# ViliamVadocz/takzero

Measured on AMD Instinct MI355X. Metric: mcts_simulations_per_s, higher is better.
Workload: dtype f16

## Files before the change

takzero_amd/csrc/tz_capi.hip:

```cpp
#include <algorithm>
#include <array>
#include <cmath>
#include <cstdlib>
#include <cstring>
#include <vector>

#include "tz_math.h"
#include "tz_nn.h"

struct tz_search {
    SearchDev d;
    tz_net* net = nullptr;
    int device = 0;
    hipStream_t stream = nullptr;
    bool own_stream = false;
    float* noise_dev = nullptr;
    int noise_cap = 0;
    uint16_t* act_dev = nullptr;
    int32_t* i32_dev = nullptr;
    int8_t* i8_dev = nullptr;
    tz_root_info* info_dev = nullptr;
    void* child_dev = nullptr;
    size_t child_cap = 0;
    hipGraphExec_t graph[2] = {nullptr, nullptr};
    int warm[2] = {0, 0};
    uint64_t graph_gen[2] = {0, 0};
    bool use_graph = true;
    uint64_t sim_index = 0;
    LeafBatchDev lb = {};
    size_t lb_slots = 0;
    std::vector<std::array<hipEvent_t, 4>> batch_events;
    double batch_ms[3] = {0.0, 0.0, 0.0};
    uint64_t batch_rounds = 0;
    bool profile = false;
    double tree_ms = 0.0;
    uint64_t steps = 0;
    std::vector<std::pair<hipEvent_t, hipEvent_t>> tree_events;
};

namespace {

int default_capacity(int n) { return n <= 3 ? 16384 : n == 4 ? 65536 : n == 5 ? 262144 : 524288; }
// ... 31 lines not shown
        (void)hipEventDestroy(ev.second);
    }
    s->tree_events.clear();
    if (s->net) {
        for (auto& ev : s->net->conv_events) {
            float ms = 0.f;
            if (hipEventElapsedTime(&ms, ev.first, ev.second) == hipSuccess) s->net->conv_ms += ms;
            (void)hipEventDestroy(ev.first);
            (void)hipEventDestroy(ev.second);
        }
        s->net->conv_events.clear();
    }
    return TZ_OK;
}

int one_simulation_eager(tz_search* s, bool from_start, bool profile);

int one_simulation(tz_search* s, bool from_start) {
    const int gi = from_start ? 1 : 0;
    s->sim_index++;
    const bool sample = s->profile && (s->sim_index % 8 == 0);
    if (!s->use_graph || sample || s->warm[gi] < 2) {
        s->warm[gi]++;
        return one_simulation_eager(s, from_start, sample);
    }
    if (s->graph[gi] && s->net && s->graph_gen[gi] != s->net->weights_gen) {
        (void)hipGraphExecDestroy(s->graph[gi]);
        s->graph[gi] = nullptr;
    }
    if (!s->graph[gi]) {
        hipGraph_t g = nullptr;
        TZ_HIP(hipStreamBeginCapture(s->stream, hipStreamCaptureModeThreadLocal));
        const int rc = one_simulation_eager(s, from_start, false);
        const hipError_t e = hipStreamEndCapture(s->stream, &g);
        if (rc) {
            if (g) (void)hipGraphDestroy(g);
            return rc;
        }
        if (e != hipSuccess) return tz_fail(TZ_EDEVICE, std::string("hipStreamEndCapture: ") + hipGetErrorString(e));
        const hipError_t ei = hipGraphInstantiate(&s->graph[gi], g, nullptr, nullptr, 0);
        (void)hipGraphDestroy(g);
        if (ei != hipSuccess) return tz_fail(TZ_EDEVICE, std::string("hipGraphInstantiate: ") + hipGetErrorString(ei));
        s->graph_gen[gi] = s->net ? s->net->weights_gen : 0;
    }
    TZ_HIP(hipGraphLaunch(s->graph[gi], s->stream));
    return TZ_OK;
}

int one_simulation_eager(tz_search* s, bool from_start, bool profile) {
    int rc;
    hipEvent_t e0 = nullptr, e1 = nullptr, e2 = nullptr, e3 = nullptr;
    const bool saved_net_profile = s->net ? s->net->profile : false;
    if (s->net) s->net->profile = profile;
    struct Restore {
        tz_search* s;
        bool v;
        ~Restore() {
            if (s->net) s->net->profile = v;
        }
    } restore{s, saved_net_profile};
    if (profile) {
        TZ_HIP(hipEventCreate(&e0));
        TZ_HIP(hipEventCreate(&e1));
        TZ_HIP(hipEventCreate(&e2));
        TZ_HIP(hipEventCreate(&e3));
        TZ_HIP(hipEventRecord(e0, s->stream));
    }
    if ((rc = tz_tree_descend(s->d, from_start, s->stream))) return rc;
    if ((rc = tz_tree_compact_leaves(s->d, s->stream))) return rc;
    if (profile) TZ_HIP(hipEventRecord(e1, s->stream));
    NetOut out{nullptr, 0, nullptr, nullptr};
    if (s->d.agent_kind == TZ_AGENT_NET) {
        if ((rc = tz_net_forward_device(s->net, s->d.leaf_env, s->d.nn_game, s->d.nn_count, 0, s->d.batch, s->stream, &out)))
            return rc;
    }
    if (profile) TZ_HIP(hipEventRecord(e2, s->stream));
    if ((rc = tz_tree_expand(s->d, out, s->stream))) return rc;
    if (profile) {
        TZ_HIP(hipEventRecord(e3, s->stream));
        s->tree_events.push_back({e0, e1});
        s->tree_events.push_back({e2, e3});
        s->steps++;
    }
    return TZ_OK;
}

int ensure_noise(tz_search* s, int amax) {
    if ((size_t)amax * s->d.batch <= (size_t)s->noise_cap) return TZ_OK;
    if (s->noise_dev) (void)hipFree(s->noise_dev);
    s->noise_dev = nullptr;
    TZ_HIP(hipMalloc(&s->noise_dev, (size_t)amax * s->d.batch * sizeof(float)));
    s->noise_cap = amax * s->d.batch;
    return TZ_OK;
}

// ... 56 lines not shown
    s->batch_events.clear();
    return TZ_OK;
}

int one_batch_round(tz_search* s) {
    int rc;
    std::array<hipEvent_t, 4> ev = {nullptr, nullptr, nullptr, nullptr};
    if (s->profile) {
        for (hipEvent_t& e : ev) TZ_HIP(hipEventCreate(&e));
        s->batch_events.push_back(ev);
        TZ_HIP(hipEventRecord(ev[0], s->stream));
    }
    if ((rc = tz_tree_descend_batch(s->d, s->lb, s->stream))) return rc;
    if ((rc = tz_tree_compact_batch(s->d, s->lb, s->stream))) return rc;
    if (s->profile) TZ_HIP(hipEventRecord(ev[1], s->stream));
    NetOut out{nullptr, 0, nullptr, nullptr};
    if (s->d.agent_kind == TZ_AGENT_NET) {
        if ((rc = tz_net_forward_device(s->net, s->lb.env, s->lb.index, s->d.nn_count, 0, s->d.batch * s->lb.leaves, s->stream, &out)))
            return rc;
    }
    if (s->profile) TZ_HIP(hipEventRecord(ev[2], s->stream));
    if ((rc = tz_tree_expand_batch(s->d, s->lb, out, s->stream))) return rc;
    if (s->profile) TZ_HIP(hipEventRecord(ev[3], s->stream));
    return TZ_OK;
}

int ensure_child(tz_search* s, size_t bytes) {
    if (bytes <= s->child_cap) return TZ_OK;
    if (s->child_dev) (void)hipFree(s->child_dev);
    s->child_dev = nullptr;
    TZ_HIP(hipMalloc(&s->child_dev, bytes));
// ... 5 lines not shown

extern "C" {

int tz_search_create(tz_net* net, int agent_kind, int batch, int board_n, int half_komi, int node_capacity,
                     tz_search** out) {
    if (!out || batch <= 0 || board_n < 3 || board_n > 6) return tz_fail(TZ_EINVAL, "tz_search_create: bad argument");
    if (agent_kind != TZ_AGENT_NET && agent_kind != TZ_AGENT_DUMMY && agent_kind != TZ_AGENT_SIMPLE)
        return tz_fail(TZ_EINVAL, "tz_search_create: unknown agent kind");
    if (agent_kind == TZ_AGENT_NET && (!net || net->n != board_n))
        return tz_fail(TZ_EINVAL, "tz_search_create: TZ_AGENT_NET needs a network of the same board size");
    int ndev = 0;
    if (hipGetDeviceCount(&ndev) != hipSuccess || ndev == 0)
        return tz_fail(TZ_EDEVICE, "tz_search_create: no HIP device available (the HIP path has no CPU fallback)");
    tz_search* s = new tz_search();
    s->use_graph = getenv("TZ_NO_GRAPH") == nullptr;
    s->net = agent_kind == TZ_AGENT_NET ? net : nullptr;
    s->device = s->net ? s->net->device : 0;
    TZ_HIP(hipSetDevice(s->device));
    if (s->net) {
        s->stream = s->net->stream;
    } else {
        TZ_HIP(hipStreamCreate(&s->stream));
        s->own_stream = true;
    }
    SearchDev& d = s->d;
    memset(&d, 0, sizeof d);
    d.batch = batch;
    d.n = board_n;
    d.half_komi = half_komi;
    d.cap = node_capacity > 0 ? node_capacity : default_capacity(board_n);
// ... 12 lines not shown
    rc |= dev_alloc(&d.t.child0, nodes);
    rc |= dev_alloc(&d.t.nchild, nodes);
    rc |= dev_alloc(&d.t.action, nodes);
    rc |= dev_alloc(&d.bank, batch);
    rc |= dev_alloc(&d.alloc, batch);
    rc |= dev_alloc(&d.env, batch);
    rc |= dev_alloc(&d.betas, batch);
    rc |= dev_alloc(&d.traj, (size_t)batch * TZ_MAX_DEPTH);
    rc |= dev_alloc(&d.traj_len, batch);
    rc |= dev_alloc(&d.start_node, batch);
    rc |= dev_alloc(&d.leaf_kind, batch);
    rc |= dev_alloc(&d.leaf_nact, batch);
    rc |= dev_alloc(&d.leaf_act, (size_t)batch * d.max_actions);
    rc |= dev_alloc(&d.leaf_env, batch);
    rc |= dev_alloc(&d.nn_game, batch);
    rc |= dev_alloc(&d.nn_count, 1);
    rc |= dev_alloc(&d.bfs_src, (size_t)batch * d.cap);
    rc |= dev_alloc(&d.counters, 3);
    rc |= dev_alloc(&d.error_flag, 1);
    rc |= dev_alloc(&d.term_reason, batch);
    rc |= dev_alloc(&d.term_winner, batch);
    rc |= dev_alloc(&s->act_dev, batch);
    rc |= dev_alloc(&s->i32_dev, batch);
    rc |= dev_alloc(&s->i8_dev, batch);
    rc |= dev_alloc(&s->info_dev, batch);
    if (rc) {
        tz_search_destroy(s);
        return tz_fail(TZ_ENOMEM, "tz_search_create: device allocation failed (lower node_capacity or batch)");
    }
    TZ_HIP(hipMemsetAsync(d.bank, 0, batch, s->stream));
    TZ_HIP(hipMemsetAsync(d.env, 0, (size_t)batch * sizeof(tz_state), s->stream));
    TZ_HIP(hipMemsetAsync(d.leaf_env, 0, (size_t)batch * sizeof(tz_state), s->stream));
    TZ_HIP(hipMemsetAsync(d.betas, 0, batch * sizeof(float), s->stream));
    TZ_HIP(hipMemsetAsync(d.start_node, 0, batch * sizeof(int32_t), s->stream));
    TZ_HIP(hipMemsetAsync(d.counters, 0, 3 * sizeof(unsigned long long), s->stream));
    TZ_HIP(hipMemsetAsync(d.error_flag, 0, 4, s->stream));
    TZ_HIP(hipMemsetAsync(d.nn_count, 0, 4, s->stream));
    if (s->net && (rc = tz_net_ensure_batch(s->net, batch))) {
        tz_search_destroy(s);
        return rc;
    }
    if ((rc = tz_tree_restart(d, nullptr, nullptr, true, false, s->stream))) {
        tz_search_destroy(s);
        return rc;
    }
    TZ_HIP(hipStreamSynchronize(s->stream));
    *out = s;
    return TZ_OK;
}

int tz_search_destroy(tz_search* s) {
    if (!s) return TZ_OK;
    (void)hipSetDevice(s->device);
    if (s->stream) (void)hipStreamSynchronize(s->stream);
    drain_profile(s);
    for (int i = 0; i < 2; i++)
        if (s->graph[i]) (void)hipGraphExecDestroy(s->graph[i]);
    SearchDev& d = s->d;
    void* ptrs[] = {d.t.eval_tag, d.t.eval_bits, d.t.visits, d.t.prob, d.t.logit, d.t.std_dev, d.t.child0, d.t.nchild,
                    d.t.action, d.bank, d.alloc, d.env, d.betas, d.traj, d.traj_len, d.start_node, d.leaf_kind,
                    d.leaf_nact, d.leaf_act, d.leaf_env, d.nn_game, d.nn_count, d.bfs_src, d.counters, d.error_flag,
                    d.term_reason, d.term_winner,
                    s->noise_dev, s->act_dev, s->i32_dev, s->i8_dev, s->info_dev, s->child_dev};
    for (void* p : ptrs)
        if (p) (void)hipFree(p);
    free_leaf_batch(s);
    drain_batch_profile(s);
    if (s->own_stream && s->stream) (void)hipStreamDestroy(s->stream);
    delete s;
    return TZ_OK;
}

int tz_search_set_positions(tz_search* s, int count, const int32_t* game_idx, const tz_state* states) {
    if (!s || count < 0 || (count && (!game_idx || !states))) return tz_fail(TZ_EINVAL, "tz_search_set_positions: bad argument");
    if (count == 0) return TZ_OK;
    TZ_HIP(hipSetDevice(s->device));
// ... 24 lines not shown
    if (!s || !opening_choice) return tz_fail(TZ_EINVAL, "tz_search_new_openings: null argument");
    TZ_HIP(hipSetDevice(s->device));
    for (int g = 0; g < s->d.batch; g++)
        if (opening_choice[g] < 0 || opening_choice[g] >= 16) return tz_fail(TZ_EINVAL, "opening choice must be in [0,16)");
    TZ_HIP(hipMemcpyAsync(s->i32_dev, opening_choice, s->d.batch * sizeof(int32_t), hipMemcpyHostToDevice, s->stream));
    int rc = tz_tree_restart(s->d, s->i32_dev, nullptr, true, true, s->stream);
    if (rc) return rc;
    TZ_HIP(hipStreamSynchronize(s->stream));
    return TZ_OK;
}

int tz_search_simulate(tz_search* s, const float* betas, int n_sims) {
    if (!s || !betas || n_sims < 0) return tz_fail(TZ_EINVAL, "tz_search_simulate: bad argument");
    TZ_HIP(hipSetDevice(s->device));
    TZ_HIP(hipMemcpyAsync(s->d.betas, betas, s->d.batch * sizeof(float), hipMemcpyHostToDevice, s->stream));
    for (int i = 0; i < n_sims; i++) {
        int rc = one_simulation(s, false);
        if (rc) return rc;
    }
    int rc = check_error_flag(s);
    drain_profile(s);
    return rc;
}

int tz_search_simulate_batch(tz_search* s, const float* betas, int leaves, int rounds) {
    if (!s || !betas || leaves < 1 || rounds < 0) return tz_fail(TZ_EINVAL, "tz_search_simulate_batch: bad argument");
    if ((long long)s->d.batch * leaves > TZ_SIMULATE_BATCH_MAX_SLOTS)
        return tz_fail(TZ_EINVAL, "tz_search_simulate_batch: batch * leaves exceeds TZ_SIMULATE_BATCH_MAX_SLOTS");
    TZ_HIP(hipSetDevice(s->device));
    int rc = ensure_leaf_batch(s, leaves);
    if (rc) return rc;
    TZ_HIP(hipMemcpyAsync(s->d.betas, betas, s->d.batch * sizeof(float), hipMemcpyHostToDevice, s->stream));
    for (int i = 0; i < rounds; i++)
        if ((rc = one_batch_round(s))) return rc;
    rc = check_error_flag(s);
    drain_batch_profile(s);
    return rc;
}

int tz_search_set_selection(tz_search* s, int rule) {
    if (!s) return tz_fail(TZ_EINVAL, "tz_search_set_selection: null argument");
    if (rule != TZ_SELECT_PUCT && rule != TZ_SELECT_UCT && rule != TZ_SELECT_IMPROVED)
        return tz_fail(TZ_EINVAL, "tz_search_set_selection: unknown selection rule");
    TZ_HIP(hipSetDevice(s->device));
    TZ_HIP(hipStreamSynchronize(s->stream));
    for (int i = 0; i < 2; i++) {
        if (s->graph[i]) (void)hipGraphExecDestroy(s->graph[i]);
        s->graph[i] = nullptr;
        s->warm[i] = 0;
    }
    s->d.select_rule = rule;
    return TZ_OK;
}

int tz_search_get_selection(tz_search* s, int* rule_out) {
    if (!s || !rule_out) return tz_fail(TZ_EINVAL, "tz_search_get_selection: null argument");
    *rule_out = s->d.select_rule;
    return TZ_OK;
}

int tz_search_batch_profile(tz_search* s, double* forward_ms, double* net_ms, double* backward_ms, uint64_t* rounds) {
// ... 444 lines not shown
```

takzero_amd/csrc/tz_engine.h:

```cpp
#pragma once
#include <hip/hip_runtime.h>
#include <stdint.h>

#include <string>
#include <vector>

#include "../../include/takzero_hip.h"

#define TZ_MAX_DEPTH 512

void tz_set_error(const std::string& msg);
int tz_fail(int code, const std::string& msg);
#define TZ_HIP(call)                                                                              \
    do {                                                                                          \
        hipError_t _e = (call);                                                                   \
        if (_e != hipSuccess)                                                                     \
            return tz_fail(TZ_EDEVICE, std::string(#call) + ": " + hipGetErrorString(_e));       \
    } while (0)

struct TreeArrays {
    uint8_t* eval_tag;
    uint32_t* eval_bits;
    uint32_t* visits;
    float* prob;
// ... 9 lines not shown
    int strict_capacity;
    int select_rule;
    TreeArrays t;
    uint8_t* bank;
    uint32_t* alloc;
    tz_state* env;
    float* betas;
    uint32_t* traj;
    uint32_t* traj_len;
    int32_t* start_node;
    uint8_t* leaf_kind;
    uint16_t* leaf_nact;
    uint16_t* leaf_act;
    tz_state* leaf_env;
    int32_t* nn_game;
    int32_t* nn_count;
    uint32_t* bfs_src;
    unsigned long long* counters;
    int32_t* error_flag;
    int8_t* term_reason;
    uint8_t* term_winner;
};

struct LeafBatchDev {
    int leaves;
    tz_state* env;
    uint16_t* act;
    uint16_t* nact;
    uint32_t* traj;
    uint32_t* traj_len;
// ... 1 lines not shown
    float* prob;
    float* value;
    float* variance;
    uint8_t* bad;
    int32_t* count;
    int32_t* forwards;
    int32_t* offset;
    int32_t* index;
};

struct NetOut {
    const float* policy;
    int policy_stride;
    const float* value;
    const float* variance;
};

int tz_tree_descend(const SearchDev& s, bool from_start_nodes, hipStream_t st);
int tz_tree_compact_leaves(const SearchDev& s, hipStream_t st);
int tz_tree_expand(const SearchDev& s, const NetOut& out, hipStream_t st);
int tz_tree_apply_noise(const SearchDev& s, const float* noise_dev, int amax, float ratio, hipStream_t st);
int tz_tree_root_info(const SearchDev& s, tz_root_info* out_dev, hipStream_t st);
int tz_tree_root_children(const SearchDev& s, int amax, uint16_t* move_idx, uint32_t* visits, uint8_t* eval_tag,
                          uint32_t* eval_bits, float* logit, float* prob, float* std_dev, hipStream_t st);
int tz_tree_node(const SearchDev& s, int game, const uint16_t* path_dev, int len, uint32_t* out_words, int* status, int amax,
                 uint16_t* move_idx, uint32_t* visits, uint8_t* eval_tag, uint32_t* eval_bits, float* logit, float* prob, float* std_dev,
                 hipStream_t st);
int tz_tree_select_best(const SearchDev& s, uint16_t* out_dev, hipStream_t st);
int tz_tree_step(const SearchDev& s, const uint16_t* actions_dev, hipStream_t st);
int tz_tree_restart(const SearchDev& s, const int32_t* choice_dev, int8_t* terminal_dev, bool force_all,
                    bool with_opening_moves, hipStream_t st);
int tz_tree_reset_games(const SearchDev& s, const int32_t* idx_dev, int count, hipStream_t st);
int tz_tree_set_start_children(const SearchDev& s, const int32_t* child_index_dev, hipStream_t st);
int tz_tree_gumbel_root_fixup(const SearchDev& s, hipStream_t st);
int tz_tree_principal_variation(const SearchDev& s, int game, uint16_t* moves_dev, int cap, int* len_dev, hipStream_t st);
// ... 5 lines not shown
```

takzero_amd/csrc/tz_nn.h:

```cpp
#pragma once
#include <string>
#include <vector>

#include "tz_engine.h"
#include "tz_ot.h"

struct ConvW {
    int taps = 0, cin = 0, cin_pad = 0, cout = 0, cout_pad = 0;
    uint16_t* w_mfma = nullptr;
    uint16_t* w_lo = nullptr;
    unsigned char* w8 = nullptr;
    float c8_scale = 0.0f;
    float* w_f32 = nullptr;
    float* bias = nullptr;
};

struct tz_net {
    int n = 0, nn = 0, arch = 0, device = 0, precision = 0, blocks = 0;
    int cin = 0, cin_pad = 0, pol_ch = 0, pol_stride = 0, ppt = 0;
    bool loaded = false, has_rnd = false, has_hash = false;
    TensorStore store;
    uint64_t weights_gen = 0;
    ConvW conv_in, policy;
    std::vector<ConvW> res;
// ... 25 lines not shown
    hipStream_t stream = nullptr;
    void* dbg_buf = nullptr;
    int dbg_groups = 0;
    void* eval_host = nullptr;
    void* eval_dev = nullptr;
    size_t eval_bytes = 0;
    hipEvent_t ev0 = nullptr, ev1 = nullptr;
    std::vector<std::pair<hipEvent_t, hipEvent_t>> conv_events;
    bool profile = false;
    double conv_ms = 0.0;
    uint64_t conv_launches = 0;
};

int tz_net_ensure_batch(tz_net* net, int batch);
int tz_net_forward_device(tz_net* net, const tz_state* states_dev, const int32_t* game_index_dev,
                          const int32_t* count_dev, int count_host, int max_positions, hipStream_t st, NetOut* out);
int tz_nn_encode_planes(int n, int cin, const tz_state* states_dev, int count, float* planes_dev, hipStream_t st);
```

takzero_amd/csrc/tz_nn.hip:

```cpp
#include "tz_nn.h"
#include "tz_fp8.h"
#include "tz_fp6.h"
#include <type_traits>
#include "tz_ot.h"

#include <algorithm>
#include <cmath>
#include <cstdio>
#include <cstdlib>
#include <cstring>
#include <atomic>
#include <map>
#include <memory>
#include <mutex>
#include <thread>

int tz_nn_launch_split(int sp, int n, const void* net_args, int max_positions, hipStream_t st);
int tz_nn_launch_c6(int n, const void* net_args, int max_positions, hipStream_t st);
size_t tz_nn_c6_seed_bytes(int n, int max_positions);

namespace {

typedef float f32x4 __attribute__((ext_vector_type(4)));
typedef unsigned int u32x4 __attribute__((ext_vector_type(4)));
// ... 2346 lines not shown
    float ss = 0.f;
    for (int sq = 0; sq < NN; sq++) ss += part[sq];
#pragma unroll
    for (int k = 0; k < PER; k++) {
        const int i = l + k * 64;
        if (i < out_stride) out[(size_t)pos * out_stride + i] = (ET)(i < in_size ? x[k] / ss : 0.f);
    }
}

__global__ __launch_bounds__(64) void rnd_finish_kernel(const float* learn, const float* target, const float* ube,
                                                        const int32_t* count_dev, int count_host, int dim, int stride,
                                                        float rmin, float rmax, float* variance) {
    const int count = count_dev ? *count_dev : count_host;
    const int pos = blockIdx.x, l = threadIdx.x;
    if (pos >= count) return;
    float s = 0.f;
    for (int i = l; i < dim; i += 64) {
        const float d = learn[(size_t)pos * stride + i] - target[(size_t)pos * stride + i];
        s += d * d;
    }
    for (int d = 32; d >= 1; d >>= 1) s += __shfl_xor(s, d);
    if (l == 0) {
        float norm = (s - rmin) / (rmax - rmin);
        norm = fminf(fmaxf(norm, 0.f), 1.f) * 4.0f;
        variance[pos] = fminf(fmaxf(fmaxf(expf(ube[pos]), norm), 0.f), 4.f);
    }
}

__global__ void plain_variance_kernel(const float* ube, const float* local, const int32_t* count_dev, int count_host,
                                      float* variance) {
    const int count = count_dev ? *count_dev : count_host;
    const int pos = blockIdx.x * blockDim.x + threadIdx.x;
    if (pos >= count) return;
    const float loc = local ? local[pos] : 0.f;
    variance[pos] = fminf(fmaxf(fmaxf(expf(ube[pos]), loc), 0.f), 4.f);
}

template <int NB>
__global__ __launch_bounds__(256) void simhash_state_kernel(const tz_state* states, const int32_t* game_index, const float* matrix,
                                                            const uint32_t* bitset, const int32_t* count_dev, int count_host, float* local,
                                                            uint32_t* index_out) {
// ... 995 lines not shown
    TZ_HIP(hipMalloc(&net->variance, batch * sizeof(float)));
    TZ_HIP(hipMalloc(&net->aux, batch * sizeof(float)));
    if (net->precision == TZ_PREC_F16C6) TZ_HIP(hipMalloc(&net->seeds, tz_nn_c6_seed_bytes(net->n, batch)));
    if (net->has_rnd) {
        const size_t in_pad = (size_t)(net->cin * net->nn + 31) / 32 * 32;
        TZ_HIP(hipMalloc(&net->rnd_in, (size_t)batch * in_pad * esz));
        TZ_HIP(hipMalloc(&net->rnd_h1, (size_t)batch * 2048 * esz));
        TZ_HIP(hipMalloc(&net->rnd_h2, (size_t)batch * 2048 * esz));
        TZ_HIP(hipMalloc(&net->rnd_out, (size_t)2 * batch * 512 * sizeof(float)));
    }
    net->max_batch = batch;
    return TZ_OK;
}

int tz_net_forward_device(tz_net* net, const tz_state* states, const int32_t* gidx, const int32_t* count_dev,
                          int count_host, int max_positions, hipStream_t st, NetOut* out) {
    if (!net->loaded) return tz_fail(TZ_ESTATE, "network has no weights loaded");
    if (max_positions > net->max_batch) return tz_fail(TZ_EINVAL, "forward: batch exceeds the network's buffers");
    int rc;
    const bool bf = net->precision != TZ_PREC_F32;
    const int nn = net->nn;
    const bool need_planes = !bf;
    if (need_planes && (rc = encode(net, states, gidx, count_dev, count_host, max_positions, st))) return rc;
    void *x = net->act_a, *t = net->act_b, *y = net->act_c;
    const bool split = prec_is_split(net->precision);
    const int rnd_in_pad = (net->cin * nn + 31) / 32 * 32;
    const bool rnd_ahead = net->eval_split && net->has_rnd && bf && net->n == 5 && net->stream_rnd;
    auto rnd_mlp = [&](hipStream_t rs) -> int {
        const bool fused_wrote_it = net->blocks > 0 && net->tower_w && (net_fused_mode() == 2 || split) && net_fused_writes_rnd_input(net);
        switch (net->n) {
            case 5:
// ... 100 lines not shown
                return rc;
            std::swap(fx, fy);
        }
        if ((rc = conv_f32(net, net->policy, fx, FILTERS, count_dev, count_host, max_positions, nullptr, net->policy_out,
                           net->pol_stride, false, true, st)))
            return rc;
        heads_kernel<float><<<max_positions, 64, 0, st>>>(fx, net->heads, count_dev, count_host, nn, net->value, net->ube);
    }
    if (net->has_rnd) {
        const int in_size = net->cin * nn, in_pad = (in_size + 31) / 32 * 32;
        float* outs[2] = {net->rnd_out, net->rnd_out + (size_t)net->max_batch * 512};
        if (bf) {
            if (!rnd_ahead && (rc = rnd_mlp(st))) return rc;
            if (rnd_ahead) TZ_HIP(hipStreamWaitEvent(st, net->ev_rnd, 0));
            float* o = net->rnd_out;
            rnd_finish_kernel<<<max_positions, 64, 0, st>>>(o, o + 512, net->ube, count_dev, count_host, 512, 1024, net->rnd_min,
                                                            net->rnd_max, net->variance);
        } else {
            rnd_prep_kernel<float><<<max_positions, 64, 0, st>>>(net->planes, count_dev, count_host, in_size, in_pad, (float*)net->rnd_in);
            for (int a = 0; a < 2; a++) {
                if ((rc = conv_f32(net, net->rnd[a][0], (float*)net->rnd_in, in_pad, count_dev, count_host, max_positions, nullptr,
                                   (float*)net->rnd_h1, 1024, true, false, st)))
                    return rc;
                if ((rc = conv_f32(net, net->rnd[a][1], (float*)net->rnd_h1, 1024, count_dev, count_host, max_positions, nullptr,
                                   (float*)net->rnd_h2, 1024, true, false, st)))
                    return rc;
                if ((rc = conv_f32(net, net->rnd[a][2], (float*)net->rnd_h2, 1024, count_dev, count_host, max_positions, nullptr,
                                   outs[a], 512, false, false, st)))
                    return rc;
            }
        }
        if (!bf)
            rnd_finish_kernel<<<max_positions, 64, 0, st>>>(outs[0], outs[1], net->ube, count_dev, count_host, 512, 512, net->rnd_min,
                                                            net->rnd_max, net->variance);
    } else if (net->has_hash) {
        if ((rc = launch_simhash_state(net->n, states, gidx, net->simhash, net->bitset, count_dev, count_host, max_positions, net->aux, nullptr, st)))
            return rc;
        plain_variance_kernel<<<(max_positions + 255) / 256, 256, 0, st>>>(net->ube, net->aux, count_dev, count_host, net->variance);
    } else {
        plain_variance_kernel<<<(max_positions + 255) / 256, 256, 0, st>>>(net->ube, nullptr, count_dev, count_host, net->variance);
    }
    hipError_t e = hipGetLastError();
    if (e != hipSuccess) return tz_fail(TZ_EDEVICE, std::string("forward launch: ") + hipGetErrorString(e));
    out->policy = net->policy_out;
    out->policy_stride = net->pol_stride;
    out->value = net->value;
    out->variance = net->variance;
    return TZ_OK;
}

extern "C" {

int tz_device_count(void) {
    int n = 0;
    if (hipGetDeviceCount(&n) != hipSuccess) return 0;
    return n;
}

int tz_net_create(int board_n, int arch, int device_id, int precision, int blocks, tz_net** out) {
    if (!out) return tz_fail(TZ_EINVAL, "tz_net_create: null out");
    int n = board_n;
    if (arch == TZ_ARCH_NET5) n = 5;
// ... 877 lines not shown
```

takzero_amd/csrc/tz_tree.hip:

```cpp
#include "tz_engine.h"
#include "tz_math.h"
#include "tz_tak_dev.h"

using namespace tzd;

namespace {

struct Ev {
    uint32_t tag, bits;
};
__device__ __forceinline__ Ev ev_value(float v) { return Ev{TZ_EVAL_VALUE, tz_float_to_bits(v)}; }
__device__ __forceinline__ bool ev_known(Ev e) { return e.tag != TZ_EVAL_VALUE; }
__device__ __forceinline__ Ev ev_negate(Ev e) {
    switch (e.tag) {
        case TZ_EVAL_VALUE: return ev_value(-tz_bits_to_float(e.bits));
        case TZ_EVAL_WIN: return Ev{TZ_EVAL_LOSS, e.bits + 1};
        case TZ_EVAL_DRAW: return Ev{TZ_EVAL_DRAW, e.bits + 1};
        default: return Ev{TZ_EVAL_WIN, e.bits + 1};
    }
}
__device__ __forceinline__ float ev_to_f32(Ev e) {
    const float base = tz_powif(TZ_DISCOUNT, e.tag == TZ_EVAL_VALUE ? 0 : (int)e.bits);
    const float x = e.tag == TZ_EVAL_VALUE ? tz_bits_to_float(e.bits)
                    : e.tag == TZ_EVAL_WIN ? 1.0f
// ... 268 lines not shown
                best_score = os;
                best_i = oi;
            }
        }
        if (best_i < 0) {
            if (l == 0) atomicMax(s.error_flag, 4);
            return 2;
        }
        node = c0 + (uint32_t)best_i;
        apply_move<N>(&env, s.t.action[base + node]);
        __syncthreads();
    }
}

template <int N, int RULE>
__global__ __launch_bounds__(64) void descend_kernel(SearchDev s, int from_start) {
    constexpr int NN = N * N;
    const int g = blockIdx.x, l = lane_id();
    __shared__ tz_state env;
    __shared__ uint32_t tnode[TZ_MAX_DEPTH];
    __shared__ uint32_t tvis[TZ_MAX_DEPTH];
    __shared__ uint8_t reach[NN * 4];
    float* prow = nullptr;
    if constexpr (RULE == TZ_SELECT_IMPROVED) {
        __shared__ float row[SelectRow<N, RULE>::LEN];
        prow = row;
    }
    load_state(&env, &s.env[g]);
    const size_t base = slab_base(s, s.bank[g], g);
    uint32_t node = 0;
    float beta = s.betas[g];
    if (from_start) {
        node = (uint32_t)s.start_node[g];
        beta = 0.0f;
    }
    __syncthreads();
    if (from_start && node != 0) {
        apply_move<N>(&env, s.t.action[base + node]);
        __syncthreads();
    }
    int depth = 0;
    Ev known{0, 0};
// ... 16 lines not shown
    }
    uint16_t* acts = s.leaf_act + (size_t)g * s.max_actions;
    const int nact = gen_moves<N>(&env, reach, acts, s.max_actions);
    if (nact > s.max_actions && l == 0) atomicMax(s.error_flag, 3);
    {
        const uint32_t* a = reinterpret_cast<const uint32_t*>(&env);
        uint32_t* b = reinterpret_cast<uint32_t*>(&s.leaf_env[g]);
        for (int i = l; i < (int)(sizeof(tz_state) / 4); i += 64) b[i] = a[i];
    }
    for (int i = l; i < depth; i += 64) s.traj[(size_t)g * TZ_MAX_DEPTH + i] = tnode[i];
    if (l == 0) {
        s.leaf_kind[g] = 1;
        s.leaf_nact[g] = (uint16_t)(nact > s.max_actions ? s.max_actions : nact);
        s.traj_len[g] = (uint32_t)depth;
    }
}

__global__ __launch_bounds__(1024) void compact_kernel(SearchDev s) {
    __shared__ int wsum[16];
    __shared__ int carry;
    const int tid = threadIdx.x, l = tid & 63, w = tid >> 6;
    if (tid == 0) carry = 0;
    __syncthreads();
    for (int chunk = 0; chunk < s.batch; chunk += 1024) {
        const int g = chunk + tid;
        const int f = (g < s.batch && s.leaf_kind[g] == 1) ? 1 : 0;
        const int incl = wave_incl_scan(f);
        if (l == 63) wsum[w] = incl;
        __syncthreads();
        int off = carry;
        for (int i = 0; i < w; i++) off += wsum[i];
        if (f) s.nn_game[off + incl - 1] = g;
        __syncthreads();
        if (tid == 1023) carry = off + incl;
        __syncthreads();
    }
    if (tid == 0) {
        *s.nn_count = carry;
        s.counters[0] += (unsigned long long)s.batch;
        s.counters[1] += (unsigned long long)carry;
    }
}

template <int N>
__global__ __launch_bounds__(64) void expand_kernel(SearchDev s, NetOut out) {
    constexpr int NN = N * N;
    const int slot = blockIdx.x, l = lane_id();
    if (slot >= *s.nn_count) return;
    const int g = s.nn_game[slot];
    extern __shared__ __attribute__((aligned(16))) unsigned char smem[];
    uint32_t* tnode = reinterpret_cast<uint32_t*>(smem);
    uint32_t* tvis = tnode + TZ_MAX_DEPTH;
    float* lg = reinterpret_cast<float*>(tvis + TZ_MAX_DEPTH);
    float* ex = lg + s.max_actions;
    const size_t base = slab_base(s, s.bank[g], g);
    const int len = (int)s.traj_len[g];
    for (int i = l; i < len; i += 64) {
        const uint32_t nd = s.traj[(size_t)g * TZ_MAX_DEPTH + i];
        tnode[i] = nd;
        tvis[i] = s.t.visits[base + nd];
    }
    const int nact = s.leaf_nact[g];
    const uint16_t* acts = s.leaf_act + (size_t)g * s.max_actions;
    float value = 0.0f, variance = 0.0f;
    if (s.agent_kind == TZ_AGENT_NET) {
        value = out.value[slot];
        variance = out.variance[slot];
    } else if (s.agent_kind == TZ_AGENT_SIMPLE) {
        __shared__ tz_state le;
        load_state(&le, &s.leaf_env[g]);
        __syncthreads();
        const int fd = flat_diff<N>(&le) - s.half_komi / 2;
        value = (float)fd / (float)NN;
        if (le.to_move == 1) value = -value;
    }
    bool nan = false;
    float mx = -3.4028235e38f;
    for (int i = l; i < nact; i += 64) {
        const int a = acts[i];
        float x;
        if (s.agent_kind == TZ_AGENT_NET) {
            x = out.policy[((size_t)slot * NN + (a % NN)) * out.policy_stride + a / NN];
// ... 2 lines not shown
        } else {
            const int ch = a / NN;
            x = ch == 0 ? 4.0f : ch == 1 ? 2.0f : ch == 2 ? 3.0f : 1.0f;
        }
        nan = nan || !(x == x);
        lg[i] = x;
        mx = x > mx ? x : mx;
    }
#pragma unroll
    for (int d = 32; d >= 1; d >>= 1) {
        const float o = __shfl_xor(mx, d);
        mx = o > mx ? o : mx;
    }
    if (__any(nan) || !(value == value) || !(variance == variance)) {
        if (l == 0) atomicMax(s.error_flag, 7);
        return;
    }
    for (int i = l; i < nact; i += 64) ex[i] = tz_expf(lg[i] - mx);
    __syncthreads();
    float sum = 0.0f;
    for (int i = 0; i < nact; i++) sum = sum + ex[i];
    const uint32_t leaf = tnode[len - 1];
    const float n = (float)tvis[len - 1];
    float mean = tz_bits_to_float(s.t.eval_bits[base + leaf]);
    mean = mean + (-mean + value) / n;
    float sd = s.t.std_dev[base + leaf];
    sd = sd + (-sd + sqrtf(variance)) / n;
    const uint32_t c0 = s.alloc[g];
    const bool full = c0 + (uint32_t)nact > (uint32_t)s.cap;
    if (full && s.strict_capacity) {
        if (l == 0) atomicMax(s.error_flag, 1);
        return;
    }
    const uint32_t child_bits = tz_float_to_bits(-mean);
    for (int i = l; i < (full ? 0 : nact); i += 64) {
        const size_t ci = base + c0 + i;
        s.t.eval_tag[ci] = TZ_EVAL_VALUE;
        s.t.eval_bits[ci] = child_bits;
        s.t.visits[ci] = 0;
        s.t.prob[ci] = ex[i] / sum;
        s.t.logit[ci] = lg[i];
        s.t.std_dev[ci] = sd;
        s.t.child0[ci] = 0;
        s.t.nchild[ci] = 0;
        s.t.action[ci] = acts[i];
    }
    if (l == 0) {
        s.t.eval_bits[base + leaf] = tz_float_to_bits(mean);
        s.t.std_dev[base + leaf] = sd;
        if (full) {
            atomicAdd(&s.counters[2], 1ull);
        } else {
            s.alloc[g] = c0 + (uint32_t)nact;
            s.t.child0[base + leaf] = c0;
            s.t.nchild[base + leaf] = (uint16_t)nact;
        }
    }
    __syncthreads();
    backup(s, base, tnode, tvis, len - 1, ev_value(value * TZ_DISCOUNT), variance * TZ_DISCOUNT * TZ_DISCOUNT, ev_value(mean));
}

template <int N, int RULE>
__global__ __launch_bounds__(64) void descend_batch_kernel(SearchDev s, LeafBatchDev b) {
    constexpr int NN = N * N;
    const int g = blockIdx.x, l = lane_id();
    __shared__ tz_state root_env;
    __shared__ tz_state env;
    __shared__ uint32_t tnode[TZ_MAX_DEPTH];
    __shared__ uint32_t tvis[TZ_MAX_DEPTH];
    __shared__ uint8_t reach[NN * 4];
    float* prow = nullptr;
    if constexpr (RULE == TZ_SELECT_IMPROVED) {
        __shared__ float row[SelectRow<N, RULE>::LEN];
        prow = row;
    }
// ... 679 lines not shown
    TZ_DISPATCH_N(s.n, TZ_DISPATCH_RULE(s.select_rule, (descend_kernel<NB, RB><<<s.batch, 64, 0, st>>>(s, from_start_nodes ? 1 : 0))));
    TZ_LAUNCH_CHECK();
    return TZ_OK;
}
int tz_tree_compact_leaves(const SearchDev& s, hipStream_t st) {
    compact_kernel<<<1, 1024, 0, st>>>(s);
    TZ_LAUNCH_CHECK();
    return TZ_OK;
}
int tz_tree_expand(const SearchDev& s, const NetOut& out, hipStream_t st) {
    const size_t smem = 2 * TZ_MAX_DEPTH * sizeof(uint32_t) + 2 * (size_t)s.max_actions * sizeof(float);
    TZ_DISPATCH_N(s.n, (expand_kernel<NB><<<s.batch, 64, smem, st>>>(s, out)));
    TZ_LAUNCH_CHECK();
    return TZ_OK;
}
int tz_tree_apply_noise(const SearchDev& s, const float* noise_dev, int amax, float ratio, hipStream_t st) {
    noise_kernel<<<s.batch, 64, 0, st>>>(s, noise_dev, amax, ratio);
    TZ_LAUNCH_CHECK();
    return TZ_OK;
}
int tz_tree_root_info(const SearchDev& s, tz_root_info* out_dev, hipStream_t st) {
    TZ_DISPATCH_N(s.n, (root_info_kernel<NB><<<s.batch, 64, 0, st>>>(s, out_dev)));
    TZ_LAUNCH_CHECK();
    return TZ_OK;
}
int tz_tree_root_children(const SearchDev& s, int amax, uint16_t* move_idx, uint32_t* visits, uint8_t* eval_tag,
                          uint32_t* eval_bits, float* logit, float* prob, float* std_dev, hipStream_t st) {
    root_children_kernel<<<s.batch, 64, 0, st>>>(s, amax, move_idx, visits, eval_tag, eval_bits, logit, prob, std_dev);
    TZ_LAUNCH_CHECK();
    return TZ_OK;
// ... 70 lines not shown
```

Before: 1.472 million.

## Fuse expand with next descend and defer RND variance into tree step

Restructures the simulation loop so that the expand of one simulation and the descend of the next run in a single tree_step kernel per game, captured as a middle graph between a head descend and a tail expand. The RND variance finish kernel is skipped and its reduction is computed inside the expand body from raw RND outputs. A new nn_slot array maps each game to its network slot. This removes one or two kernel launches and a pass over global memory per simulation, in exchange for a heavier kernel launched on every game and more shared memory per block.

```diff
diff --git a/takzero_amd/csrc/tz_capi.hip b/takzero_amd/csrc/tz_capi.hip
--- a/takzero_amd/csrc/tz_capi.hip
+++ b/takzero_amd/csrc/tz_capi.hip
@@ -22,10 +22,11 @@
     tz_root_info* info_dev = nullptr;
     void* child_dev = nullptr;
     size_t child_cap = 0;
-    hipGraphExec_t graph[2] = {nullptr, nullptr};
-    int warm[2] = {0, 0};
-    uint64_t graph_gen[2] = {0, 0};
+    hipGraphExec_t graph[3] = {nullptr, nullptr, nullptr};
+    int warm[3] = {0, 0, 0};
+    uint64_t graph_gen[3] = {0, 0, 0};
     bool use_graph = true;
+    bool tree_step = true;
     uint64_t sim_index = 0;
     LeafBatchDev lb = {};
     size_t lb_slots = 0;
@@ -87,7 +88,33 @@
     return TZ_OK;
 }
 
-int one_simulation_eager(tz_search* s, bool from_start, bool profile);
+enum SimPart { SIM_WHOLE, SIM_HEAD, SIM_MIDDLE, SIM_TAIL };
+
+int simulation_part_eager(tz_search* s, SimPart part, bool from_start, bool profile);
+
+int simulation_part_graph(tz_search* s, int gi, SimPart part, bool from_start) {
+    if (s->graph[gi] && s->net && s->graph_gen[gi] != s->net->weights_gen) {
+        (void)hipGraphExecDestroy(s->graph[gi]);
+        s->graph[gi] = nullptr;
+    }
+    if (!s->graph[gi]) {
+        hipGraph_t g = nullptr;
+        TZ_HIP(hipStreamBeginCapture(s->stream, hipStreamCaptureModeThreadLocal));
+        const int rc = simulation_part_eager(s, part, from_start, false);
+        const hipError_t e = hipStreamEndCapture(s->stream, &g);
+        if (rc) {
+            if (g) (void)hipGraphDestroy(g);
+            return rc;
+        }
+        if (e != hipSuccess) return tz_fail(TZ_EDEVICE, std::string("hipStreamEndCapture: ") + hipGetErrorString(e));
+        const hipError_t ei = hipGraphInstantiate(&s->graph[gi], g, nullptr, nullptr, 0);
+        (void)hipGraphDestroy(g);
+        if (ei != hipSuccess) return tz_fail(TZ_EDEVICE, std::string("hipGraphInstantiate: ") + hipGetErrorString(ei));
+        s->graph_gen[gi] = s->net ? s->net->weights_gen : 0;
+    }
+    TZ_HIP(hipGraphLaunch(s->graph[gi], s->stream));
+    return TZ_OK;
+}
 
 int one_simulation(tz_search* s, bool from_start) {
     const int gi = from_start ? 1 : 0;
@@ -95,32 +122,32 @@
     const bool sample = s->profile && (s->sim_index % 8 == 0);
     if (!s->use_graph || sample || s->warm[gi] < 2) {
         s->warm[gi]++;
-        return one_simulation_eager(s, from_start, sample);
-    }
-    if (s->graph[gi] && s->net && s->graph_gen[gi] != s->net->weights_gen) {
-        (void)hipGraphExecDestroy(s->graph[gi]);
-        s->graph[gi] = nullptr;
-    }
-    if (!s->graph[gi]) {
-        hipGraph_t g = nullptr;
-        TZ_HIP(hipStreamBeginCapture(s->stream, hipStreamCaptureModeThreadLocal));
-        const int rc = one_simulation_eager(s, from_start, false);
-        const hipError_t e = hipStreamEndCapture(s->stream, &g);
-        if (rc) {
-            if (g) (void)hipGraphDestroy(g);
-            return rc;
-        }
-        if (e != hipSuccess) return tz_fail(TZ_EDEVICE, std::string("hipStreamEndCapture: ") + hipGetErrorString(e));
-        const hipError_t ei = hipGraphInstantiate(&s->graph[gi], g, nullptr, nullptr, 0);
-        (void)hipGraphDestroy(g);
-        if (ei != hipSuccess) return tz_fail(TZ_EDEVICE, std::string("hipGraphInstantiate: ") + hipGetErrorString(ei));
-        s->graph_gen[gi] = s->net ? s->net->weights_gen : 0;
-    }
-    TZ_HIP(hipGraphLaunch(s->graph[gi], s->stream));
-    return TZ_OK;
-}
-
-int one_simulation_eager(tz_search* s, bool from_start, bool profile) {
+        return simulation_part_eager(s, SIM_WHOLE, from_start, sample);
+    }
+    return simulation_part_graph(s, gi, SIM_WHOLE, from_start);
+}
+
+int simulations_tree_step(tz_search* s, int n) {
+    int rc;
+    auto sampled = [&](uint64_t index) { return s->profile && (index % 8 == 0); };
+    if ((rc = simulation_part_eager(s, SIM_HEAD, false, sampled(s->sim_index + 1)))) return rc;
+    for (int i = 0; i < n; i++) {
+        s->sim_index++;
+        const bool sample = sampled(s->sim_index);
+        if (i == n - 1) {
+            rc = simulation_part_eager(s, SIM_TAIL, false, sample);
+        } else if (!s->use_graph || sample || s->warm[2] < 2) {
+            s->warm[2]++;
+            rc = simulation_part_eager(s, SIM_MIDDLE, false, sample);
+        } else {
+            rc = simulation_part_graph(s, 2, SIM_MIDDLE, false);
+        }
+        if (rc) return rc;
+    }
+    return TZ_OK;
+}
+
+int simulation_part_eager(tz_search* s, SimPart part, bool from_start, bool profile) {
     int rc;
     hipEvent_t e0 = nullptr, e1 = nullptr, e2 = nullptr, e3 = nullptr;
     const bool saved_net_profile = s->net ? s->net->profile : false;
@@ -132,26 +159,39 @@
             if (s->net) s->net->profile = v;
         }
     } restore{s, saved_net_profile};
+    if (part == SIM_WHOLE || part == SIM_HEAD) {
+        if (profile) {
+            TZ_HIP(hipEventCreate(&e0));
+            TZ_HIP(hipEventCreate(&e1));
+            TZ_HIP(hipEventRecord(e0, s->stream));
+        }
+        if ((rc = tz_tree_descend(s->d, from_start, s->stream))) return rc;
+        if ((rc = tz_tree_compact_leaves(s->d, s->stream))) return rc;
+        if (profile) {
+            TZ_HIP(hipEventRecord(e1, s->stream));
+            s->tree_events.push_back({e0, e1});
+        }
+        if (part == SIM_HEAD) return TZ_OK;
+    }
+    NetOut out{};
+    if (s->d.agent_kind == TZ_AGENT_NET) {
+        if ((rc = tz_net_forward_device(s->net, s->d.leaf_env, s->d.nn_game, s->d.nn_count, 0, s->d.batch, s->stream, &out,
+                                        s->tree_step)))
+            return rc;
+    }
     if (profile) {
-        TZ_HIP(hipEventCreate(&e0));
-        TZ_HIP(hipEventCreate(&e1));
         TZ_HIP(hipEventCreate(&e2));
         TZ_HIP(hipEventCreate(&e3));
-        TZ_HIP(hipEventRecord(e0, s->stream));
-    }
-    if ((rc = tz_tree_descend(s->d, from_start, s->stream))) return rc;
-    if ((rc = tz_tree_compact_leaves(s->d, s->stream))) return rc;
-    if (profile) TZ_HIP(hipEventRecord(e1, s->stream));
-    NetOut out{nullptr, 0, nullptr, nullptr};
-    if (s->d.agent_kind == TZ_AGENT_NET) {
-        if ((rc = tz_net_forward_device(s->net, s->d.leaf_env, s->d.nn_game, s->d.nn_count, 0, s->d.batch, s->stream, &out)))
-            return rc;
-    }
-    if (profile) TZ_HIP(hipEventRecord(e2, s->stream));
-    if ((rc = tz_tree_expand(s->d, out, s->stream))) return rc;
+        TZ_HIP(hipEventRecord(e2, s->stream));
+    }
+    if (part == SIM_MIDDLE) {
+        if ((rc = tz_tree_expand_descend(s->d, out, s->stream))) return rc;
+        if ((rc = tz_tree_compact_leaves(s->d, s->stream))) return rc;
+    } else {
+        if ((rc = tz_tree_expand(s->d, out, s->stream))) return rc;
+    }
     if (profile) {
         TZ_HIP(hipEventRecord(e3, s->stream));
-        s->tree_events.push_back({e0, e1});
         s->tree_events.push_back({e2, e3});
         s->steps++;
     }
@@ -238,7 +278,7 @@
     if ((rc = tz_tree_descend_batch(s->d, s->lb, s->stream))) return rc;
     if ((rc = tz_tree_compact_batch(s->d, s->lb, s->stream))) return rc;
     if (s->profile) TZ_HIP(hipEventRecord(ev[1], s->stream));
-    NetOut out{nullptr, 0, nullptr, nullptr};
+    NetOut out{};
     if (s->d.agent_kind == TZ_AGENT_NET) {
         if ((rc = tz_net_forward_device(s->net, s->lb.env, s->lb.index, s->d.nn_count, 0, s->d.batch * s->lb.leaves, s->stream, &out)))
             return rc;
@@ -274,6 +314,10 @@
         return tz_fail(TZ_EDEVICE, "tz_search_create: no HIP device available (the HIP path has no CPU fallback)");
     tz_search* s = new tz_search();
     s->use_graph = getenv("TZ_NO_GRAPH") == nullptr;
+    {
+        const char* ts = getenv("TZ_TREE_STEP");
+        s->tree_step = !(ts && ts[0] == '0' && ts[1] == 0);
+    }
     s->net = agent_kind == TZ_AGENT_NET ? net : nullptr;
     s->device = s->net ? s->net->device : 0;
     TZ_HIP(hipSetDevice(s->device));
@@ -316,6 +360,7 @@
     rc |= dev_alloc(&d.leaf_act, (size_t)batch * d.max_actions);
     rc |= dev_alloc(&d.leaf_env, batch);
     rc |= dev_alloc(&d.nn_game, batch);
+    rc |= dev_alloc(&d.nn_slot, batch);
     rc |= dev_alloc(&d.nn_count, 1);
     rc |= dev_alloc(&d.bfs_src, (size_t)batch * d.cap);
     rc |= dev_alloc(&d.counters, 3);
@@ -338,6 +383,7 @@
     TZ_HIP(hipMemsetAsync(d.counters, 0, 3 * sizeof(unsigned long long), s->stream));
     TZ_HIP(hipMemsetAsync(d.error_flag, 0, 4, s->stream));
     TZ_HIP(hipMemsetAsync(d.nn_count, 0, 4, s->stream));
+    TZ_HIP(hipMemsetAsync(d.nn_slot, 0, batch * sizeof(int32_t), s->stream));
     if (s->net && (rc = tz_net_ensure_batch(s->net, batch))) {
         tz_search_destroy(s);
         return rc;
@@ -356,12 +402,12 @@
     (void)hipSetDevice(s->device);
     if (s->stream) (void)hipStreamSynchronize(s->stream);
     drain_profile(s);
-    for (int i = 0; i < 2; i++)
+    for (int i = 0; i < 3; i++)
         if (s->graph[i]) (void)hipGraphExecDestroy(s->graph[i]);
     SearchDev& d = s->d;
     void* ptrs[] = {d.t.eval_tag, d.t.eval_bits, d.t.visits, d.t.prob, d.t.logit, d.t.std_dev, d.t.child0, d.t.nchild,
                     d.t.action, d.bank, d.alloc, d.env, d.betas, d.traj, d.traj_len, d.start_node, d.leaf_kind,
-                    d.leaf_nact, d.leaf_act, d.leaf_env, d.nn_game, d.nn_count, d.bfs_src, d.counters, d.error_flag,
+                    d.leaf_nact, d.leaf_act, d.leaf_env, d.nn_game, d.nn_slot, d.nn_count, d.bfs_src, d.counters, d.error_flag,
                     d.term_reason, d.term_winner,
                     s->noise_dev, s->act_dev, s->i32_dev, s->i8_dev, s->info_dev, s->child_dev};
     for (void* p : ptrs)
@@ -416,11 +462,14 @@
     if (!s || !betas || n_sims < 0) return tz_fail(TZ_EINVAL, "tz_search_simulate: bad argument");
     TZ_HIP(hipSetDevice(s->device));
     TZ_HIP(hipMemcpyAsync(s->d.betas, betas, s->d.batch * sizeof(float), hipMemcpyHostToDevice, s->stream));
-    for (int i = 0; i < n_sims; i++) {
-        int rc = one_simulation(s, false);
-        if (rc) return rc;
-    }
-    int rc = check_error_flag(s);
+    int rc;
+    if (s->tree_step && n_sims >= 2) {
+        if ((rc = simulations_tree_step(s, n_sims))) return rc;
+    } else {
+        for (int i = 0; i < n_sims; i++)
+            if ((rc = one_simulation(s, false))) return rc;
+    }
+    rc = check_error_flag(s);
     drain_profile(s);
     return rc;
 }
@@ -446,7 +495,7 @@
         return tz_fail(TZ_EINVAL, "tz_search_set_selection: unknown selection rule");
     TZ_HIP(hipSetDevice(s->device));
     TZ_HIP(hipStreamSynchronize(s->stream));
-    for (int i = 0; i < 2; i++) {
+    for (int i = 0; i < 3; i++) {
         if (s->graph[i]) (void)hipGraphExecDestroy(s->graph[i]);
         s->graph[i] = nullptr;
         s->warm[i] = 0;
diff --git a/takzero_amd/csrc/tz_engine.h b/takzero_amd/csrc/tz_engine.h
--- a/takzero_amd/csrc/tz_engine.h
+++ b/takzero_amd/csrc/tz_engine.h
@@ -47,6 +47,7 @@
     uint16_t* leaf_act;
     tz_state* leaf_env;
     int32_t* nn_game;
+    int32_t* nn_slot;
     int32_t* nn_count;
     uint32_t* bfs_src;
     unsigned long long* counters;
@@ -78,11 +79,16 @@
     int policy_stride;
     const float* value;
     const float* variance;
+    const float* rnd_out;
+    const float* ube;
+    int rnd_dim, rnd_stride;
+    float rnd_min, rnd_max;
 };
 
 int tz_tree_descend(const SearchDev& s, bool from_start_nodes, hipStream_t st);
 int tz_tree_compact_leaves(const SearchDev& s, hipStream_t st);
 int tz_tree_expand(const SearchDev& s, const NetOut& out, hipStream_t st);
+int tz_tree_expand_descend(const SearchDev& s, const NetOut& out, hipStream_t st);
 int tz_tree_apply_noise(const SearchDev& s, const float* noise_dev, int amax, float ratio, hipStream_t st);
 int tz_tree_root_info(const SearchDev& s, tz_root_info* out_dev, hipStream_t st);
 int tz_tree_root_children(const SearchDev& s, int amax, uint16_t* move_idx, uint32_t* visits, uint8_t* eval_tag,
diff --git a/takzero_amd/csrc/tz_nn.h b/takzero_amd/csrc/tz_nn.h
--- a/takzero_amd/csrc/tz_nn.h
+++ b/takzero_amd/csrc/tz_nn.h
@@ -63,5 +63,6 @@
 
 int tz_net_ensure_batch(tz_net* net, int batch);
 int tz_net_forward_device(tz_net* net, const tz_state* states_dev, const int32_t* game_index_dev,
-                          const int32_t* count_dev, int count_host, int max_positions, hipStream_t st, NetOut* out);
+                          const int32_t* count_dev, int count_host, int max_positions, hipStream_t st, NetOut* out,
+                          bool defer_rnd_variance = false);
 int tz_nn_encode_planes(int n, int cin, const tz_state* states_dev, int count, float* planes_dev, hipStream_t st);
diff --git a/takzero_amd/csrc/tz_nn.hip b/takzero_amd/csrc/tz_nn.hip
--- a/takzero_amd/csrc/tz_nn.hip
+++ b/takzero_amd/csrc/tz_nn.hip
@@ -1,4 +1,5 @@
 #include "tz_nn.h"
+#include "tz_rnd_variance.h"
 #include "tz_fp8.h"
 #include "tz_fp6.h"
 #include <type_traits>
@@ -2384,17 +2385,8 @@
     const int count = count_dev ? *count_dev : count_host;
     const int pos = blockIdx.x, l = threadIdx.x;
     if (pos >= count) return;
-    float s = 0.f;
-    for (int i = l; i < dim; i += 64) {
-        const float d = learn[(size_t)pos * stride + i] - target[(size_t)pos * stride + i];
-        s += d * d;
-    }
-    for (int d = 32; d >= 1; d >>= 1) s += __shfl_xor(s, d);
-    if (l == 0) {
-        float norm = (s - rmin) / (rmax - rmin);
-        norm = fminf(fmaxf(norm, 0.f), 1.f) * 4.0f;
-        variance[pos] = fminf(fmaxf(fmaxf(expf(ube[pos]), norm), 0.f), 4.f);
-    }
+    const float v = tz_rnd_variance(learn + (size_t)pos * stride, target + (size_t)pos * stride, ube[pos], dim, rmin, rmax, l);
+    if (l == 0) variance[pos] = v;
 }
 
 __global__ void plain_variance_kernel(const float* ube, const float* local, const int32_t* count_dev, int count_host,
@@ -3420,7 +3412,7 @@
 }
 
 int tz_net_forward_device(tz_net* net, const tz_state* states, const int32_t* gidx, const int32_t* count_dev,
-                          int count_host, int max_positions, hipStream_t st, NetOut* out) {
+                          int count_host, int max_positions, hipStream_t st, NetOut* out, bool defer_rnd_variance) {
     if (!net->loaded) return tz_fail(TZ_ESTATE, "network has no weights loaded");
     if (max_positions > net->max_batch) return tz_fail(TZ_EINVAL, "forward: batch exceeds the network's buffers");
     int rc;
@@ -3551,8 +3543,9 @@
             if (!rnd_ahead && (rc = rnd_mlp(st))) return rc;
             if (rnd_ahead) TZ_HIP(hipStreamWaitEvent(st, net->ev_rnd, 0));
             float* o = net->rnd_out;
-            rnd_finish_kernel<<<max_positions, 64, 0, st>>>(o, o + 512, net->ube, count_dev, count_host, 512, 1024, net->rnd_min,
-                                                            net->rnd_max, net->variance);
+            if (!defer_rnd_variance)
+                rnd_finish_kernel<<<max_positions, 64, 0, st>>>(o, o + 512, net->ube, count_dev, count_host, 512, 1024, net->rnd_min,
+                                                                net->rnd_max, net->variance);
         } else {
             rnd_prep_kernel<float><<<max_positions, 64, 0, st>>>(net->planes, count_dev, count_host, in_size, in_pad, (float*)net->rnd_in);
             for (int a = 0; a < 2; a++) {
@@ -3583,6 +3576,16 @@
     out->policy_stride = net->pol_stride;
     out->value = net->value;
     out->variance = net->variance;
+    out->rnd_out = nullptr;
+    out->ube = net->ube;
+    out->rnd_dim = 512;
+    out->rnd_stride = 1024;
+    out->rnd_min = net->rnd_min;
+    out->rnd_max = net->rnd_max;
+    if (defer_rnd_variance && net->has_rnd && bf) {
+        out->variance = nullptr;
+        out->rnd_out = net->rnd_out;
+    }
     return TZ_OK;
 }
 
diff --git a/takzero_amd/csrc/tz_rnd_variance.h b/takzero_amd/csrc/tz_rnd_variance.h
--- /dev/null
+++ b/takzero_amd/csrc/tz_rnd_variance.h
@@ -0,0 +1,15 @@
+#pragma once
+#include <hip/hip_runtime.h>
+
+__device__ __forceinline__ float tz_rnd_variance(const float* learn, const float* target, float ube, int dim, float rmin,
+                                                 float rmax, int lane) {
+    float s = 0.f;
+    for (int i = lane; i < dim; i += 64) {
+        const float d = learn[i] - target[i];
+        s = __builtin_fmaf(d, d, s);
+    }
+    for (int d = 32; d >= 1; d >>= 1) s += __shfl_xor(s, d);
+    float norm = (s - rmin) / (rmax - rmin);
+    norm = fminf(fmaxf(norm, 0.f), 1.f) * 4.0f;
+    return fminf(fmaxf(fmaxf(expf(ube), norm), 0.f), 4.f);
+}
diff --git a/takzero_amd/csrc/tz_tree.hip b/takzero_amd/csrc/tz_tree.hip
--- a/takzero_amd/csrc/tz_tree.hip
+++ b/takzero_amd/csrc/tz_tree.hip
@@ -1,5 +1,6 @@
 #include "tz_engine.h"
 #include "tz_math.h"
+#include "tz_rnd_variance.h"
 #include "tz_tak_dev.h"
 
 using namespace tzd;
@@ -306,18 +307,9 @@
 }
 
 template <int N, int RULE>
-__global__ __launch_bounds__(64) void descend_kernel(SearchDev s, int from_start) {
-    constexpr int NN = N * N;
-    const int g = blockIdx.x, l = lane_id();
-    __shared__ tz_state env;
-    __shared__ uint32_t tnode[TZ_MAX_DEPTH];
-    __shared__ uint32_t tvis[TZ_MAX_DEPTH];
-    __shared__ uint8_t reach[NN * 4];
-    float* prow = nullptr;
-    if constexpr (RULE == TZ_SELECT_IMPROVED) {
-        __shared__ float row[SelectRow<N, RULE>::LEN];
-        prow = row;
-    }
+__device__ __forceinline__ void descend_body(const SearchDev& s, int g, int from_start, tz_state& env, uint32_t* tnode, uint32_t* tvis,
+                                             uint8_t* reach, float* prow) {
+    const int l = lane_id();
     load_state(&env, &s.env[g]);
     const size_t base = slab_base(s, s.bank[g], g);
     uint32_t node = 0;
@@ -364,6 +356,21 @@
         s.leaf_nact[g] = (uint16_t)(nact > s.max_actions ? s.max_actions : nact);
         s.traj_len[g] = (uint32_t)depth;
     }
+}
+
+template <int N, int RULE>
+__global__ __launch_bounds__(64) void descend_kernel(SearchDev s, int from_start) {
+    constexpr int NN = N * N;
+    __shared__ tz_state env;
+    __shared__ uint32_t tnode[TZ_MAX_DEPTH];
+    __shared__ uint32_t tvis[TZ_MAX_DEPTH];
+    __shared__ uint8_t reach[NN * 4];
+    float* prow = nullptr;
+    if constexpr (RULE == TZ_SELECT_IMPROVED) {
+        __shared__ float row[SelectRow<N, RULE>::LEN];
+        prow = row;
+    }
+    descend_body<N, RULE>(s, blockIdx.x, from_start, env, tnode, tvis, reach, prow);
 }
 
 __global__ __launch_bounds__(1024) void compact_kernel(SearchDev s) {
@@ -380,7 +387,10 @@
         __syncthreads();
         int off = carry;
         for (int i = 0; i < w; i++) off += wsum[i];
-        if (f) s.nn_game[off + incl - 1] = g;
+        if (f) {
+            s.nn_game[off + incl - 1] = g;
+            s.nn_slot[g] = off + incl - 1;
+        }
         __syncthreads();
         if (tid == 1023) carry = off + incl;
         __syncthreads();
@@ -393,16 +403,10 @@
 }
 
 template <int N>
-__global__ __launch_bounds__(64) void expand_kernel(SearchDev s, NetOut out) {
+__device__ __forceinline__ bool expand_body(const SearchDev& s, const NetOut& out, int g, int slot, uint32_t* tnode, uint32_t* tvis,
+                                            float* lg, float* ex) {
     constexpr int NN = N * N;
-    const int slot = blockIdx.x, l = lane_id();
-    if (slot >= *s.nn_count) return;
-    const int g = s.nn_game[slot];
-    extern __shared__ __attribute__((aligned(16))) unsigned char smem[];
-    uint32_t* tnode = reinterpret_cast<uint32_t*>(smem);
-    uint32_t* tvis = tnode + TZ_MAX_DEPTH;
-    float* lg = reinterpret_cast<float*>(tvis + TZ_MAX_DEPTH);
-    float* ex = lg + s.max_actions;
+    const int l = lane_id();
     const size_t base = slab_base(s, s.bank[g], g);
     const int len = (int)s.traj_len[g];
     for (int i = l; i < len; i += 64) {
@@ -415,7 +419,10 @@
     float value = 0.0f, variance = 0.0f;
     if (s.agent_kind == TZ_AGENT_NET) {
         value = out.value[slot];
-        variance = out.variance[slot];
+        variance = out.rnd_out ? tz_rnd_variance(out.rnd_out + (size_t)slot * out.rnd_stride,
+                                                 out.rnd_out + (size_t)slot * out.rnd_stride + out.rnd_dim, out.ube[slot], out.rnd_dim,
+                                                 out.rnd_min, out.rnd_max, l)
+                               : out.variance[slot];
     } else if (s.agent_kind == TZ_AGENT_SIMPLE) {
         __shared__ tz_state le;
         load_state(&le, &s.leaf_env[g]);
@@ -448,7 +455,7 @@
     }
     if (__any(nan) || !(value == value) || !(variance == variance)) {
         if (l == 0) atomicMax(s.error_flag, 7);
-        return;
+        return false;
     }
     for (int i = l; i < nact; i += 64) ex[i] = tz_expf(lg[i] - mx);
     __syncthreads();
@@ -464,7 +471,7 @@
     const bool full = c0 + (uint32_t)nact > (uint32_t)s.cap;
     if (full && s.strict_capacity) {
         if (l == 0) atomicMax(s.error_flag, 1);
-        return;
+        return false;
     }
     const uint32_t child_bits = tz_float_to_bits(-mean);
     for (int i = l; i < (full ? 0 : nact); i += 64) {
@@ -492,7 +499,51 @@
     }
     __syncthreads();
     backup(s, base, tnode, tvis, len - 1, ev_value(value * TZ_DISCOUNT), variance * TZ_DISCOUNT * TZ_DISCOUNT, ev_value(mean));
-}
+    return true;
+}
+
+template <int N>
+__global__ __launch_bounds__(64) void expand_kernel(SearchDev s, NetOut out) {
+    const int slot = blockIdx.x;
+    if (slot >= *s.nn_count) return;
+    extern __shared__ __attribute__((aligned(16))) unsigned char smem[];
+    uint32_t* tnode = reinterpret_cast<uint32_t*>(smem);
+    uint32_t* tvis = tnode + TZ_MAX_DEPTH;
+    float* lg = reinterpret_cast<float*>(tvis + TZ_MAX_DEPTH);
+    float* ex = lg + s.max_actions;
+    expand_body<N>(s, out, s.nn_game[slot], slot, tnode, tvis, lg, ex);
+}
+
+template <int N, int RULE>
+__global__ __launch_bounds__(64) void tree_step_kernel(SearchDev s, NetOut out) {
+    constexpr int NN = N * N;
+    const int g = blockIdx.x, l = lane_id();
+    __shared__ tz_state env;
+    __shared__ uint32_t tnode[TZ_MAX_DEPTH];
+    __shared__ uint32_t tvis[TZ_MAX_DEPTH];
+    __shared__ uint8_t reach[NN * 4];
+    extern __shared__ __attribute__((aligned(16))) unsigned char smem[];
+    float* lg = reinterpret_cast<float*>(smem);
+    float* ex = lg + s.max_actions;
+    float* prow = nullptr;
+    if constexpr (RULE == TZ_SELECT_IMPROVED) {
+        __shared__ float row[SelectRow<N, RULE>::LEN];
+        prow = row;
+    }
+    if (s.leaf_kind[g] == 1) {
+        if (!expand_body<N>(s, out, g, s.nn_slot[g], tnode, tvis, lg, ex)) {
+            if (l == 0) {
+                s.leaf_kind[g] = 0;
+                s.traj_len[g] = 0;
+            }
+            return;
+        }
+        __threadfence_block();
+        __syncthreads();
+    }
+    descend_body<N, RULE>(s, g, 0, env, tnode, tvis, reach, prow);
+}
+
 
 template <int N, int RULE>
 __global__ __launch_bounds__(64) void descend_batch_kernel(SearchDev s, LeafBatchDev b) {
@@ -1202,6 +1253,12 @@
     TZ_LAUNCH_CHECK();
     return TZ_OK;
 }
+int tz_tree_expand_descend(const SearchDev& s, const NetOut& out, hipStream_t st) {
+    const size_t smem = 2 * (size_t)s.max_actions * sizeof(float);
+    TZ_DISPATCH_N(s.n, TZ_DISPATCH_RULE(s.select_rule, (tree_step_kernel<NB, RB><<<s.batch, 64, smem, st>>>(s, out))));
+    TZ_LAUNCH_CHECK();
+    return TZ_OK;
+}
 int tz_tree_apply_noise(const SearchDev& s, const float* noise_dev, int amax, float ratio, hipStream_t st) {
     noise_kernel<<<s.batch, 64, 0, st>>>(s, noise_dev, amax, ratio);
     TZ_LAUNCH_CHECK();
```

Result: no change. 1.476 million (median of 6 runs) (+0.3%).
